# autonomousvision/connecting_the_dots

Hardware: AMD Instinct MI355X
Metric: Mpix*disparities/s on 512x432x128 cost volume; disparity MAE vs ref (higher is better)
Workload: dtype f32

## Files before the change

connecting_the_dots_amd/csrc/argmax_rerank.hip:

```cpp
#include "ctd_internal.h"
#include "ctd_ncc_point.h"
#include "ctd_rank.h"
#include "ctd_tail.h"


namespace ctd {

constexpr int kScanBatch = 8;
template <int PX>
__global__ __launch_bounds__(256) __attribute__((amdgpu_waves_per_eu(5, 8))) void argmax_scan_kernel(const float* __restrict__ vol, int64_t* __restrict__ idx,
                                                          float* __restrict__ best, int D, long HW, int W,
                                                          int bs, float eps, long total_threads, WorkList work) {
  const long t = (long)blockIdx.x * blockDim.x + threadIdx.x;
  if (t >= total_threads) return;
  const long p0 = t * PX;
  const long f = p0 / HW, q0 = p0 - f * HW;
  const float* v = vol + f * D * HW + q0;
  const int w0 = (int)(q0 % W);
  float v0[PX], v1[PX];
  int i0[PX], dc[PX];
#pragma unroll
  for (int k = 0; k < PX; ++k) { v0[k] = -INFINITY; v1[k] = -INFINITY; i0[k] = 0; dc[k] = w0 + k + (bs - 1 - bs / 2); }
  constexpr int kBatch = kScanBatch;
  const bool wave_masks = __any(dc[0] < D - 1);
  for (int d0 = 0; d0 < D; d0 += kBatch) {
    float x[kBatch][PX];
#pragma unroll
    for (int u = 0; u < kBatch; ++u) {
      const float* src = v + (long)min(d0 + u, D - 1) * HW;
      if constexpr (PX == 4) {
        typedef float f4 __attribute__((ext_vector_type(4)));
        const f4 q = __builtin_nontemporal_load((const f4*)src);
        x[u][0] = q.x; x[u][1] = q.y; x[u][2] = q.z; x[u][3] = q.w;
      } else if constexpr (PX == 2) {
        typedef float f2 __attribute__((ext_vector_type(2)));
        const f2 q = __builtin_nontemporal_load((const f2*)src);
        x[u][0] = q.x; x[u][1] = q.y;
      } else {
        x[u][0] = __builtin_nontemporal_load(src);
      }
    }
    if (wave_masks || d0 + kBatch > D) {
#pragma unroll
      for (int u = 0; u < kBatch; ++u) {
        const int d = d0 + u;
#pragma unroll
        for (int k = 0; k < PX; ++k) {
          const float y = (d > dc[k] || d >= D) ? -INFINITY : x[u][k];
          v1[k] = __builtin_amdgcn_fmed3f(v0[k], v1[k], y);
          i0[k] = y > v0[k] ? d : i0[k];
          v0[k] = fmaxf(v0[k], y);
        }
      }
    } else {
#pragma unroll
      for (int u = 0; u < kBatch; ++u) {
#pragma unroll
        for (int k = 0; k < PX; ++k) {
          const float y = x[u][k];
          v1[k] = __builtin_amdgcn_fmed3f(v0[k], v1[k], y);
          i0[k] = y > v0[k] ? d0 + u : i0[k];
          v0[k] = fmaxf(v0[k], y);
        }
      }
    }
  }
#pragma unroll
  for (int k = 0; k < PX; ++k) {
    const bool hard = v1[k] >= v0[k] - eps;
    idx[p0 + k] = hard ? (int64_t)(-1 - i0[k]) : (int64_t)i0[k];
    if (best) best[p0 + k] = v0[k];
    if (hard) work.list[atomicAdd(work.counters, 1u)] = p0 + k;
  }
}

constexpr int kMaskWords = 8;

__device__ inline float wave_maxf(float v) {
#pragma unroll
  for (int o = 32; o > 0; o >>= 1) v = fmaxf(v, __shfl_xor(v, o));
  return v;
}

struct RunSource {
  const float* run_vals;
  const float* v1;
  int W1, xoff, per_frame;
};

template <int WORDS, bool VOL>
__device__ __forceinline__ void resolve_role(float* lds_resolve, const float* __restrict__ vol, const float* __restrict__ in0,
                                             const float* __restrict__ in1, long in1_frame_stride,
                                             int64_t* __restrict__ idx, float* __restrict__ best, int D, int H, int W, int bs,
                                             float eps, WorkList work, RunSource rsrc, unsigned role_block,
                                             unsigned n_role_blocks, unsigned waves_used = 4, unsigned* stamp = nullptr) {
  if ((threadIdx.x >> 6) >= waves_used) return;
  const int lane = threadIdx.x & 63;
  const int half = bs / 2, span = bs + D - 1;
  float* sA = lds_resolve + (threadIdx.x >> 6) * 2 * (bs * bs + bs * span);
  float* sB = sA + bs * bs;
  float* sAq = sB + bs * span;
  float* sBq = sAq + bs * bs;
  const float bs2f = (float)(bs * bs);
  const long HW = (long)H * W;
  unsigned seg_cnt[kWorkListParts];
  unsigned longest = 0;
#pragma unroll
  for (int k = 0; k < kWorkListParts; ++k) seg_cnt[k] = work.counters[min(k, work.parts - 1) * kWorkListStride];
#pragma unroll
  for (int k = 0; k < kWorkListParts; ++k) {
    if (k >= work.parts) seg_cnt[k] = 0u;
    longest = max(longest, seg_cnt[k]);
  }
  const unsigned n_slots = longest * (unsigned)work.parts;
  CTD_POST_STAMP_S(stamp, 1, longest);
  const unsigned n_waves = n_role_blocks * waves_used;
  for (unsigned slot = role_block * waves_used + (threadIdx.x >> 6); slot < n_slots; slot += n_waves) {
    const unsigned seg = slot & (unsigned)(work.parts - 1), entry = slot / (unsigned)work.parts;
    unsigned cnt = 0;
#pragma unroll
    for (int k = 0; k < kWorkListParts; ++k) cnt = seg == (unsigned)k ? seg_cnt[k] : cnt;
    if (entry >= cnt) continue;
    const long pj = work.list[(long)seg * work.seg_cap + entry];
    CTD_POST_STAMP_S(stamp, 2, pj);
    CTD_POST_STAMP_ITEM(stamp);
    const long fj = pj / HW, qj = pj - fj * HW;
    const int hj = (int)(qj / W), wj = (int)(qj - (long)hj * W);
    const float* v = VOL ? vol + fj * D * HW + qj : nullptr;
    const int d_clamped = wj + (bs - 1 - bs / 2);
    unsigned long long mask[WORDS];
    int n_cand = 0;
    float x[WORDS];
    bool run_listed = false;
    float rv = 0.f;
    if constexpr (VOL) {
      if (rsrc.run_vals && d_clamped < D) {
        const long z = rsrc.per_frame ? fj : 0;
        run_listed = rsrc.v1[(z * H + hj) * rsrc.W1 + (rsrc.xoff - (bs - 1 - bs / 2))] == 0.f;
        if (run_listed) rv = rsrc.run_vals[(fj * H + hj) * D + d_clamped];
      }
#pragma unroll
      for (int wd = 0; wd < WORDS; ++wd) {
        const int d = min(wd * 64 + lane, D - 1);
        x[wd] = v[(long)(rsrc.run_vals ? min(d, d_clamped) : d) * HW];
        if (run_listed && d >= d_clamped) x[wd] = rv;
      }
      CTD_POST_STAMP_V(stamp, 3, x[0]);
    }
    constexpr int kPreA = 2, kPreB = 20;
    const bool pre = !VOL && bs * bs <= 64 * kPreA && bs * span <= 64 * kPreB;
    const float* a = in0 + fj * HW;
    const float* b = in1 + fj * in1_frame_stride;
    float ta[kPreA], tb[kPreB];
    if (pre) {
#pragma unroll
      for (int k = 0; k < kPreA; ++k) {
        const int i = min(lane + 64 * k, bs * bs - 1);
        const int bh = i / bs, bw = i - bh * bs;
        ta[k] = a[(long)clampi(hj + bh - half, 0, H - 1) * W + clampi(wj + bw - half, 0, W - 1)];
      }
#pragma unroll
      for (int k = 0; k < kPreB; ++k) {
        const int i = min(lane + 64 * k, bs * span - 1);
        const int bh = i / span, c = i - bh * span;
        tb[k] = b[(long)clampi(hj + bh - half, 0, H - 1) * W + clampi(wj - half - (D - 1) + c, 0, W - 1)];
      }
    }
    if constexpr (VOL) {
      float m = -INFINITY;
#pragma unroll
      for (int wd = 0; wd < WORDS; ++wd)
        if (wd * 64 + lane < D && wd * 64 + lane <= d_clamped) m = fmaxf(m, x[wd]);
      m = wave_maxf(m);
      bool have_clamped = false;
#pragma unroll
      for (int wd = 0; wd < WORDS; ++wd) {
        unsigned long long bits = __ballot(wd * 64 + lane < D && x[wd] >= m - eps);
        const int c0 = d_clamped - wd * 64;
        if (c0 < 64) {
          const unsigned long long run = c0 <= 0 ? bits : bits & ~((1ull << c0) - 1ull);
          bits &= ~run;
          if (!have_clamped && run) {
            bits |= run & (0ull - run);
            have_clamped = true;
          }
        }
        mask[wd] = bits;
        n_cand += __popcll(bits);
      }
    } else {
#pragma unroll
      for (int wd = 0; wd < WORDS; ++wd) {
        const int last = min(D - 1, d_clamped) - wd * 64;
        mask[wd] = last < 0 ? 0ull : (last >= 63 ? ~0ull : ((1ull << (last + 1)) - 1ull));
        n_cand += __popcll(mask[wd]);
      }
    }
    float eb = 0.f;
    int ei = 0x7fffffff;
    const bool rescore = VOL ? n_cand > 1 : n_cand >= 1;
    if (rescore && pre) {
#pragma unroll
      for (int k = 0; k < kPreA; ++k)
        if (lane + 64 * k < bs * bs) {
          sA[lane + 64 * k] = ta[k];
          sAq[lane + 64 * k] = ta[k] / bs2f;
        }
#pragma unroll
      for (int k = 0; k < kPreB; ++k)
        if (lane + 64 * k < bs * span) {
          sB[lane + 64 * k] = tb[k];
          sBq[lane + 64 * k] = tb[k] / bs2f;
        }
    } else if (rescore) {
      for (int i = lane; i < bs * bs; i += 64) {
        const int bh = i / bs, bw = i - bh * bs;
        const float xa = a[(long)clampi(hj + bh - half, 0, H - 1) * W + clampi(wj + bw - half, 0, W - 1)];
        sA[i] = xa;
        sAq[i] = xa / bs2f;
      }
      constexpr int NB = 20;
      for (int i0 = lane; i0 < bs * span; i0 += 64 * NB) {
        float t[NB];
#pragma unroll
        for (int k = 0; k < NB; ++k) {
          const int i = min(i0 + 64 * k, bs * span - 1);
          const int bh = i / span, c = i - bh * span;
          t[k] = b[(long)clampi(hj + bh - half, 0, H - 1) * W + clampi(wj - half - (D - 1) + c, 0, W - 1)];
        }
#pragma unroll
        for (int k = 0; k < NB; ++k)
          if (i0 + 64 * k < bs * span) {
            sB[i0 + 64 * k] = t[k];
            sBq[i0 + 64 * k] = t[k] / bs2f;
          }
      }
    }
    CTD_POST_STAMP(stamp, 4);
    if (rescore) {
      for (int c0 = 0; c0 < n_cand; c0 += 64) {
        int my_d = -1, k = 0;
#pragma unroll
        for (int wd = 0; wd < WORDS; ++wd) {
          unsigned long long mj = mask[wd];
          if (k + __popcll(mj) <= c0 || k >= c0 + 64) { k += __popcll(mj); continue; }
          while (mj) {
            const int d = wd * 64 + __ffsll((long long)mj) - 1;
            mj &= mj - 1;
            if (k - c0 == lane) my_d = d;
            ++k;
          }
        }
        float e = -INFINITY;
        if (my_d >= 0) e = bs == 9 ? ncc_exact_point_lds_bs<9>(sA, sB, sAq, sBq, span, (D - 1) - my_d)
                                   : ncc_exact_point_lds(sA, sB, bs, span, (D - 1) - my_d);
        const float em = wave_maxf(e);
        const unsigned long long holders = __ballot(my_d >= 0 && e == em);
        const int dl = __shfl(my_d, holders ? __ffsll((long long)holders) - 1 : 0);
        if (ei == 0x7fffffff || em > eb) { eb = em; ei = dl; }
      }
    } else {
#pragma unroll
      for (int wd = 0; wd < WORDS; ++wd)
        if (mask[wd]) ei = min(ei, wd * 64 + __ffsll((long long)mask[wd]) - 1);
    }
    CTD_POST_STAMP_S(stamp, 5, ei);
    if (lane == 0) {
      idx[pj] = ei;
      if (best) {
        if constexpr (VOL) best[pj] = (run_listed && ei >= d_clamped) ? rv : v[(long)(rsrc.run_vals ? min(ei, d_clamped) : ei) * HW];
        else if (rescore) best[pj] = eb;
      }
    }
    CTD_POST_STAMP(stamp, 6);
    CTD_POST_STAMP(stamp, 9);
    stamp = nullptr;
  }
}

template <int WORDS, bool VOL>
__global__ __launch_bounds__(256) void argmax_resolve_kernel(const float* __restrict__ vol, const float* __restrict__ in0,
                                                             const float* __restrict__ in1, long in1_frame_stride,
                                                             int64_t* __restrict__ idx, float* __restrict__ best, int D,
                                                             int H, int W, int bs, float eps, WorkList work) {
  extern __shared__ float lds_dyn[];
  resolve_role<WORDS, VOL>(lds_dyn, vol, in0, in1, in1_frame_stride, idx, best, D, H, W, bs, eps, work,
                           RunSource{nullptr, nullptr, 0, 0, 0}, blockIdx.x, gridDim.x);
}

constexpr long kResolveBlocks = 1024;
constexpr unsigned kTailResolveWaves = 2;

template <int WORDS, bool VOL>
__global__ __launch_bounds__(256) void rank_tail_kernel(float* __restrict__ vol, const float* __restrict__ in0,
                                                        const float* __restrict__ in1, long in1_frame_stride,
                                                        int64_t* __restrict__ idx, float* __restrict__ best,
                                                        const unsigned char* __restrict__ flags, int frames, int D, int H,
                                                        int W, int bs, float eps, WorkList work, RunSource rsrc,
                                                        unsigned* __restrict__ counters,
                                                        const unsigned long long* __restrict__ run_rows,
                                                        const unsigned long long* __restrict__ flag_a,
                                                        const unsigned long long* __restrict__ flag_b, unsigned n_resolve,
                                                        unsigned n_runs, unsigned n_decode) {
  extern __shared__ float lds_dyn[];
  const unsigned n_pair = min(n_resolve, n_runs);
  unsigned role, rb;
  if (blockIdx.x < n_decode) { role = 2; rb = blockIdx.x; }
  else {
    const unsigned b = blockIdx.x - n_decode;
    if (b < 2 * n_pair) { role = b & 1; rb = b >> 1; }
    else { role = n_resolve > n_runs ? 0 : 1; rb = b - n_pair; }
  }
  if (blockIdx.x == 0 && threadIdx.x == 0) counters[0] = 0u;
  unsigned* stamp = CTD_POST_STAMP_SLOT(role);
  if (role == 0) {
    resolve_role<WORDS, VOL>(lds_dyn, vol, in0, in1, in1_frame_stride, idx, best, D, H, W, bs, eps, work, rsrc, rb, n_resolve,
                             kTailResolveWaves, stamp);
  } else if (role == 1) {
    if constexpr (VOL)
      runs_role(vol, rsrc.run_vals, counters, run_rows, rsrc.per_frame, 1, H, W, D, bs, (int)(rb >> 2), (int)(rb & 3), 4,
                (int*)lds_dyn, stamp);
  } else {
    decode_role((unsigned long long*)idx, best, flags, counters, flag_a, flag_b, rsrc.per_frame, frames, H, W, D,
                rb * 4 + (threadIdx.x >> 6), n_decode * 4, stamp);
  }
}


CTD_POST_STAMP_EXPORT(ctd_debug_read_tail_stamps)

template <bool VOL>
static int launch_resolve(const float* vol, const float* in0, const float* in1, long in1_frame_stride, int64_t* idx,
                          float* best, long total, int D, int H, int W, int bs, float eps, const WorkList& work,
                          hipStream_t stream) {
  const size_t lds = sizeof(float) * 4 * 2 * ((size_t)bs * bs + (size_t)bs * (bs + D - 1));
  if (lds > 160 * 1024) return CTD_ERR_UNSUPPORTED;
  const long chunks = (total + 255) / 256;
  auto resolve = D <= 128 ? argmax_resolve_kernel<2, VOL> : (D <= 256 ? argmax_resolve_kernel<4, VOL> : argmax_resolve_kernel<8, VOL>);
  if (lds > 64 * 1024)
    CTD_HIP_TRY(hipFuncSetAttribute((const void*)resolve, hipFuncAttributeMaxDynamicSharedMemorySize, (int)lds));
  hipLaunchKernelGGL(resolve, dim3((unsigned)(chunks < kResolveBlocks ? chunks : kResolveBlocks)), dim3(256), lds, stream, vol,
                     in0, in1, in1_frame_stride, idx, best, D, H, W, bs, eps, work);
  CTD_LAUNCH_CHECK();
  return CTD_OK;
}

template <bool VOL>
static int launch_tail(const RankPlan& rp, float* vol, const float* in0, const float* in1, long in1_frame_stride,
                       int64_t* idx, float* best, int frames, int D, int H, int W, int bs, hipStream_t stream) {
  size_t lds = sizeof(float) * kTailResolveWaves * 2 * ((size_t)bs * bs + (size_t)bs * (bs + D - 1));
  if (lds < sizeof(int) * (size_t)H) lds = sizeof(int) * (size_t)H;
  if (lds > 160 * 1024) return CTD_ERR_UNSUPPORTED;
  const long total = (long)frames * H * W;
  const long chunks = (total + 255) / 256;
  const unsigned n_resolve = rp.eps >= 0.f ? (unsigned)(chunks < kResolveBlocks ? chunks : kResolveBlocks) : 0u;
  const unsigned n_runs = VOL ? (unsigned)(frames * ceil_div(D, kRunPlanes)) * 4u : 0u;
  const unsigned n_decode = 128u;
  auto kern = D <= 128 ? rank_tail_kernel<2, VOL> : (D <= 256 ? rank_tail_kernel<4, VOL> : rank_tail_kernel<8, VOL>);
  if (lds > 64 * 1024)
    CTD_HIP_TRY(hipFuncSetAttribute((const void*)kern, hipFuncAttributeMaxDynamicSharedMemorySize, (int)lds));
  const RunSource rsrc = {rp.run_vals, rp.v1, rp.W1, rp.xoff, in1_frame_stride != 0 ? 1 : 0};
  hipLaunchKernelGGL(kern, dim3(n_resolve + n_runs + n_decode), dim3(256), lds, stream, vol, in0, in1, in1_frame_stride, idx,
                     best, rp.flags, frames, D, H, W, bs, rp.eps, rp.work, rsrc, rp.counters, rp.run_rows, rp.flag_a, rp.flag_b,
                     n_resolve,
                     n_runs, n_decode);
  CTD_LAUNCH_CHECK();
  return CTD_OK;
}

int rank_tail_f32(const RankPlan& rp, float* vol, const float* in0, const float* in1, long in1_frame_stride, int64_t* idx,
                  float* best, int frames, int D, int H, int W, int bs, hipStream_t stream) {
  return vol ? launch_tail<true>(rp, vol, in0, in1, in1_frame_stride, idx, best, frames, D, H, W, bs, stream)
             : launch_tail<false>(rp, nullptr, in0, in1, in1_frame_stride, idx, best, frames, D, H, W, bs, stream);
}

int argmax_rerank_f32(const float* vol, const float* in0, const float* in1, long in1_frame_stride, int64_t* idx,
                      float* best, int frames, int D, int H, int W, int bs, float eps, void* workspace,
                      size_t workspace_bytes, bool counter_cleared, hipStream_t stream) {
  if (D > kMaskWords * 64) return CTD_ERR_UNSUPPORTED;
  const long total = (long)frames * H * W;
  const long HW = (long)H * W;
  if (!workspace || workspace_bytes < 16 + sizeof(int64_t) * (size_t)total) return CTD_ERR_WORKSPACE;
  unsigned* n_hard = (unsigned*)workspace;
  const WorkList work = {n_hard, (int64_t*)((char*)workspace + 16), 1, W, total};
  if (!counter_cleared) CTD_HIP_TRY(hipMemsetAsync(n_hard, 0, 16, stream));
  const bool vec4 = W % 4 == 0 && ((uintptr_t)vol % 16) == 0;
  const int px = vec4 ? 4 : 1;
  if (px == 4)
    hipLaunchKernelGGL(argmax_scan_kernel<4>, dim3((unsigned)((total / 4 + 255) / 256)), dim3(256), 0, stream, vol,
                       idx, best, D, HW, W, bs, eps, total / 4, work);
  else
    hipLaunchKernelGGL(argmax_scan_kernel<1>, dim3((unsigned)((total + 255) / 256)), dim3(256), 0, stream, vol, idx,
                       best, D, HW, W, bs, eps, total, work);
  CTD_LAUNCH_CHECK();
  if (eps < 0.f) return CTD_OK;
  return launch_resolve<true>(vol, in0, in1, in1_frame_stride, idx, best, total, D, H, W, bs, eps, work, stream);
}

}
```

Baseline: 1.048 million.

## Stage per-candidate windows in rounds and balance resolve work across list segments

```diff
diff --git a/connecting_the_dots_amd/csrc/argmax_rerank.hip b/connecting_the_dots_amd/csrc/argmax_rerank.hip
--- a/connecting_the_dots_amd/csrc/argmax_rerank.hip
+++ b/connecting_the_dots_amd/csrc/argmax_rerank.hip
@@ -75,6 +75,12 @@
 }
 
 constexpr int kMaskWords = 8;
+constexpr int kCandRound = 6;
+constexpr int kCandBatch = 4;
+
+__host__ __device__ inline size_t resolve_wave_floats(bool vol_path, int bs, int D) {
+  return vol_path ? (size_t)2 * bs * bs * (1 + kCandRound) : (size_t)2 * (bs * bs + bs * (bs + D - 1));
+}
 
 __device__ inline float wave_maxf(float v) {
 #pragma unroll
@@ -87,6 +93,31 @@
   const float* v1;
   int W1, xoff, per_frame;
 };
+
+__device__ __forceinline__ void stage_round_windows(float* sA, float* sAq, const float* __restrict__ a,
+                                                    const float* __restrict__ b, int bs, int my_d, int i_lo, int i_hi,
+                                                    int hj, int wj, int H, int W, int D, int lane) {
+  const int bs2 = bs * bs, half = bs / 2;
+  const float bs2f = (float)bs2;
+  for (int i0 = i_lo; i0 < i_hi; i0 += 64 * kCandBatch) {
+    float t[kCandBatch];
+#pragma unroll
+    for (int u = 0; u < kCandBatch; ++u) {
+      const int i = min(i0 + 64 * u + lane, i_hi - 1);
+      const int cj = i / bs2, r = i - cj * bs2;
+      const int bh = r / bs, bw = r - bh * bs;
+      const int c = bw + (D - 1) - __shfl(my_d, max(cj - 1, 0));
+      const int col = cj == 0 ? wj + bw - half : wj - half - (D - 1) + c;
+      t[u] = (cj == 0 ? a : b)[(long)clampi(hj + bh - half, 0, H - 1) * W + clampi(col, 0, W - 1)];
+    }
+#pragma unroll
+    for (int u = 0; u < kCandBatch; ++u)
+      if (i0 + 64 * u + lane < i_hi) {
+        sA[i0 + 64 * u + lane] = t[u];
+        sAq[i0 + 64 * u + lane] = t[u] / bs2f;
+      }
+  }
+}
 
 template <int WORDS, bool VOL>
 __device__ __forceinline__ void resolve_role(float* lds_resolve, const float* __restrict__ vol, const float* __restrict__ in0,
@@ -97,30 +128,36 @@
   if ((threadIdx.x >> 6) >= waves_used) return;
   const int lane = threadIdx.x & 63;
   const int half = bs / 2, span = bs + D - 1;
-  float* sA = lds_resolve + (threadIdx.x >> 6) * 2 * (bs * bs + bs * span);
+  const int nB = VOL ? kCandRound * bs * bs : bs * span;
+  float* sA = lds_resolve + (threadIdx.x >> 6) * resolve_wave_floats(VOL, bs, D);
   float* sB = sA + bs * bs;
-  float* sAq = sB + bs * span;
+  float* sAq = sB + nB;
   float* sBq = sAq + bs * bs;
   const float bs2f = (float)(bs * bs);
   const long HW = (long)H * W;
-  unsigned seg_cnt[kWorkListParts];
-  unsigned longest = 0;
-#pragma unroll
-  for (int k = 0; k < kWorkListParts; ++k) seg_cnt[k] = work.counters[min(k, work.parts - 1) * kWorkListStride];
-#pragma unroll
-  for (int k = 0; k < kWorkListParts; ++k) {
-    if (k >= work.parts) seg_cnt[k] = 0u;
-    longest = max(longest, seg_cnt[k]);
-  }
-  const unsigned n_slots = longest * (unsigned)work.parts;
-  CTD_POST_STAMP_S(stamp, 1, longest);
+  const unsigned my_cnt = lane < work.parts ? work.counters[lane * kWorkListStride] : 0u;
+  unsigned incl = my_cnt;
+#pragma unroll
+  for (int o = 1; o < kWorkListParts; o <<= 1) {
+    const unsigned up = __shfl_up(incl, o, kWorkListParts);
+    if ((lane & (kWorkListParts - 1)) >= o) incl += up;
+  }
+  const unsigned n_items = (unsigned)__builtin_amdgcn_readlane((int)incl, kWorkListParts - 1);
+  CTD_POST_STAMP_S(stamp, 1, n_items);
+#ifdef CTD_STAMPS
+  unsigned* const stamp_row = stamp;
+  if (stamp_row && lane == 0) stamp_row[7] = 0u;
+#endif
   const unsigned n_waves = n_role_blocks * waves_used;
-  for (unsigned slot = role_block * waves_used + (threadIdx.x >> 6); slot < n_slots; slot += n_waves) {
-    const unsigned seg = slot & (unsigned)(work.parts - 1), entry = slot / (unsigned)work.parts;
-    unsigned cnt = 0;
-#pragma unroll
-    for (int k = 0; k < kWorkListParts; ++k) cnt = seg == (unsigned)k ? seg_cnt[k] : cnt;
-    if (entry >= cnt) continue;
+  const unsigned wave0 = role_block * waves_used + (unsigned)__builtin_amdgcn_readfirstlane((int)(threadIdx.x >> 6));
+  for (unsigned g = wave0; g < n_items; g += n_waves) {
+    const unsigned j = g & (kWorkListParts - 1), q = n_items / kWorkListParts, r = n_items & (kWorkListParts - 1);
+    const unsigned k_item = j * q + min(j, r) + g / kWorkListParts;
+    const unsigned seg = (unsigned)__popcll(__ballot(lane < kWorkListParts && k_item >= incl));
+    const unsigned entry = k_item - (unsigned)__builtin_amdgcn_readlane((int)(incl - my_cnt), (int)seg);
+#ifdef CTD_STAMPS
+    if (stamp_row && lane == 0) stamp_row[7] += 1u;
+#endif
     const long pj = work.list[(long)seg * work.seg_cap + entry];
     CTD_POST_STAMP_S(stamp, 2, pj);
     CTD_POST_STAMP_ITEM(stamp);
@@ -199,7 +236,40 @@
     float eb = 0.f;
     int ei = 0x7fffffff;
     const bool rescore = VOL ? n_cand > 1 : n_cand >= 1;
-    if (rescore && pre) {
+    if constexpr (VOL) {
+      if (rescore) {
+        const int bs2 = bs * bs;
+        for (int c0 = 0; c0 < n_cand; c0 += kCandRound) {
+          int my_d = -1, k = 0;
+#pragma unroll
+          for (int wd = 0; wd < WORDS; ++wd) {
+            unsigned long long mj = mask[wd];
+            if (k + __popcll(mj) <= c0 || k >= c0 + kCandRound) { k += __popcll(mj); continue; }
+            while (mj && k < c0 + kCandRound) {
+              const int d = wd * 64 + __ffsll((long long)mj) - 1;
+              mj &= mj - 1;
+              if (k - c0 == lane) my_d = d;
+              ++k;
+            }
+            k += __popcll(mj);
+          }
+          const int i_lo = c0 == 0 ? 0 : bs2, i_hi = (1 + min(kCandRound, n_cand - c0)) * bs2;
+          stage_round_windows(sA, sAq, a, b, bs, my_d, i_lo, i_hi, hj, wj, H, W, D, lane);
+          if (c0 == 0) CTD_POST_STAMP(stamp, 4);
+          float e = -INFINITY;
+          if (my_d >= 0) e = bs == 9 ? ncc_exact_point_lds_bs<9>(sA, sB, sAq, sBq, 9, lane * 81)
+                                     : ncc_exact_point_lds(sA, sB, bs, bs, lane * bs2);
+          const float em = wave_maxf(e);
+          const unsigned long long holders = __ballot(my_d >= 0 && e == em);
+          const int dl = __shfl(my_d, holders ? __ffsll((long long)holders) - 1 : 0);
+          if (ei == 0x7fffffff || em > eb) { eb = em; ei = dl; }
+          __builtin_amdgcn_wave_barrier();
+        }
+      } else {
+        CTD_POST_STAMP(stamp, 4);
+      }
+    }
+    if (!VOL && rescore && pre) {
 #pragma unroll
       for (int k = 0; k < kPreA; ++k)
         if (lane + 64 * k < bs * bs) {
@@ -212,7 +282,7 @@
           sB[lane + 64 * k] = tb[k];
           sBq[lane + 64 * k] = tb[k] / bs2f;
         }
-    } else if (rescore) {
+    } else if (!VOL && rescore) {
       for (int i = lane; i < bs * bs; i += 64) {
         const int bh = i / bs, bw = i - bh * bs;
         const float xa = a[(long)clampi(hj + bh - half, 0, H - 1) * W + clampi(wj + bw - half, 0, W - 1)];
@@ -236,8 +306,8 @@
           }
       }
     }
-    CTD_POST_STAMP(stamp, 4);
-    if (rescore) {
+    if constexpr (!VOL) CTD_POST_STAMP(stamp, 4);
+    if (!VOL && rescore) {
       for (int c0 = 0; c0 < n_cand; c0 += 64) {
         int my_d = -1, k = 0;
 #pragma unroll
@@ -259,7 +329,7 @@
         const int dl = __shfl(my_d, holders ? __ffsll((long long)holders) - 1 : 0);
         if (ei == 0x7fffffff || em > eb) { eb = em; ei = dl; }
       }
-    } else {
+    } else if (!rescore) {
 #pragma unroll
       for (int wd = 0; wd < WORDS; ++wd)
         if (mask[wd]) ei = min(ei, wd * 64 + __ffsll((long long)mask[wd]) - 1);
@@ -289,19 +359,21 @@
 }
 
 constexpr long kResolveBlocks = 1024;
-constexpr unsigned kTailResolveWaves = 2;
+__host__ __device__ constexpr unsigned tail_resolve_waves(bool vol_path) { return vol_path ? 4u : 2u; }
+constexpr long kTailResolveBlocksVol = 512;
 
 template <int WORDS, bool VOL>
-__global__ __launch_bounds__(256) void rank_tail_kernel(float* __restrict__ vol, const float* __restrict__ in0,
-                                                        const float* __restrict__ in1, long in1_frame_stride,
-                                                        int64_t* __restrict__ idx, float* __restrict__ best,
-                                                        const unsigned char* __restrict__ flags, int frames, int D, int H,
-                                                        int W, int bs, float eps, WorkList work, RunSource rsrc,
-                                                        unsigned* __restrict__ counters,
-                                                        const unsigned long long* __restrict__ run_rows,
-                                                        const unsigned long long* __restrict__ flag_a,
-                                                        const unsigned long long* __restrict__ flag_b, unsigned n_resolve,
-                                                        unsigned n_runs, unsigned n_decode) {
+__global__ __launch_bounds__(256) __attribute__((amdgpu_num_sgpr(96)))
+void rank_tail_kernel(float* __restrict__ vol, const float* __restrict__ in0,
+                      const float* __restrict__ in1, long in1_frame_stride,
+                      int64_t* __restrict__ idx, float* __restrict__ best,
+                      const unsigned char* __restrict__ flags, int frames, int D, int H,
+                      int W, int bs, float eps, WorkList work, RunSource rsrc,
+                      unsigned* __restrict__ counters,
+                      const unsigned long long* __restrict__ run_rows,
+                      const unsigned long long* __restrict__ flag_a,
+                      const unsigned long long* __restrict__ flag_b, unsigned n_resolve,
+                      unsigned n_runs, unsigned n_decode) {
   extern __shared__ float lds_dyn[];
   const unsigned n_pair = min(n_resolve, n_runs);
   unsigned role, rb;
@@ -315,7 +387,7 @@
   unsigned* stamp = CTD_POST_STAMP_SLOT(role);
   if (role == 0) {
     resolve_role<WORDS, VOL>(lds_dyn, vol, in0, in1, in1_frame_stride, idx, best, D, H, W, bs, eps, work, rsrc, rb, n_resolve,
-                             kTailResolveWaves, stamp);
+                             tail_resolve_waves(VOL), stamp);
   } else if (role == 1) {
     if constexpr (VOL)
       runs_role(vol, rsrc.run_vals, counters, run_rows, rsrc.per_frame, 1, H, W, D, bs, (int)(rb >> 2), (int)(rb & 3), 4,
@@ -333,7 +405,7 @@
 static int launch_resolve(const float* vol, const float* in0, const float* in1, long in1_frame_stride, int64_t* idx,
                           float* best, long total, int D, int H, int W, int bs, float eps, const WorkList& work,
                           hipStream_t stream) {
-  const size_t lds = sizeof(float) * 4 * 2 * ((size_t)bs * bs + (size_t)bs * (bs + D - 1));
+  const size_t lds = sizeof(float) * 4 * resolve_wave_floats(VOL, bs, D);
   if (lds > 160 * 1024) return CTD_ERR_UNSUPPORTED;
   const long chunks = (total + 255) / 256;
   auto resolve = D <= 128 ? argmax_resolve_kernel<2, VOL> : (D <= 256 ? argmax_resolve_kernel<4, VOL> : argmax_resolve_kernel<8, VOL>);
@@ -348,12 +420,13 @@
 template <bool VOL>
 static int launch_tail(const RankPlan& rp, float* vol, const float* in0, const float* in1, long in1_frame_stride,
                        int64_t* idx, float* best, int frames, int D, int H, int W, int bs, hipStream_t stream) {
-  size_t lds = sizeof(float) * kTailResolveWaves * 2 * ((size_t)bs * bs + (size_t)bs * (bs + D - 1));
+  size_t lds = sizeof(float) * tail_resolve_waves(VOL) * resolve_wave_floats(VOL, bs, D);
   if (lds < sizeof(int) * (size_t)H) lds = sizeof(int) * (size_t)H;
   if (lds > 160 * 1024) return CTD_ERR_UNSUPPORTED;
   const long total = (long)frames * H * W;
   const long chunks = (total + 255) / 256;
-  const unsigned n_resolve = rp.eps >= 0.f ? (unsigned)(chunks < kResolveBlocks ? chunks : kResolveBlocks) : 0u;
+  const long resolve_cap = VOL ? kTailResolveBlocksVol : kResolveBlocks;
+  const unsigned n_resolve = rp.eps >= 0.f ? (unsigned)(chunks < resolve_cap ? chunks : resolve_cap) : 0u;
   const unsigned n_runs = VOL ? (unsigned)(frames * ceil_div(D, kRunPlanes)) * 4u : 0u;
   const unsigned n_decode = 128u;
   auto kern = D <= 128 ? rank_tail_kernel<2, VOL> : (D <= 256 ? rank_tail_kernel<4, VOL> : rank_tail_kernel<8, VOL>);
```

New measurement: 1.036 million. 0.988x the previous value.
